# EarthyScience/EasyHybrid.jl

Hardware: NVIDIA B200
Metric: training samples/sec (fwd+bwd+Adam) (higher is better)
Workload: dtype f32

## Files before the change

easyhybrid.jl_b200/csrc/eh_epoch_kernel.cuh:

```cuda
#pragma once
#include "eh_step_kernel.cuh"

namespace eh {

struct EpochArgs {
    const float4* rec;
    const int* idx;
    long long n;
    int B;
    long long first_step;
    int nsteps;
    int nb;
    float* pblock;
    int nflat, ntheta;
    float* m;
    float* v;
    OptState* ost;
    const int* wsrc;
    const int* pmap;
    const int* cells;
    const float* pspan;
    const int* slot_of_flat;
    const float* bscal;
    uint2* pbuf;
    int pbuf_rows;
    unsigned tag_base;
    float* stats_out;
    int npartp;
    int work_floats;
    int wcomp;
    int pg_log2;
    int tile_floats;
    int T, agg_mean;
    int loss_kind[MAXT];
    PSlot slot[MAXPS];
    float pmc[4];
    int use_bn;
    const PmProgData* prog;
    int scale_rt;
    unsigned pass_mask[3];
    int pm_id;
    int opt_kind, adamw_coupled;
    float eta, beta1, beta2, eps, lambda;
    long long* dbg;
    const unsigned* ready;
    unsigned ready_base;
    unsigned* done;
    const int* host_total;
    float* loss_stream;
    long long batch_stride;
    int world, rank;
    unsigned step_base;
    uint2* inbox_peer[EH_MAX_WORLD];
    unsigned* err;
    int stagger_ns;
    int eng_off;
};

__device__ __forceinline__ void st_volatile_v2(uint2* p, unsigned x, unsigned y)
{
    asm volatile("st.volatile.global.v2.u32 [%0], {%1, %2};" ::"l"(p), "r"(x), "r"(y) : "memory");
}
__device__ __forceinline__ uint2 ld_volatile_v2(const uint2* p)
{
    uint2 v;
    asm volatile("ld.volatile.global.v2.u32 {%0, %1}, [%2];" : "=r"(v.x), "=r"(v.y) : "l"(p) : "memory");
    return v;
}
#ifndef EH_TOT_REPL_N
#define EH_TOT_REPL_N 8
#endif
constexpr int EH_TOT_REPL = EH_TOT_REPL_N;
constexpr int EH_PBUF_EXTRA_ROWS = 32;
constexpr unsigned EH_SPIN_LIMIT = 1u << 26;

__device__ __forceinline__ void st_cg_v4(uint2* p, unsigned x0, unsigned t0, unsigned x1, unsigned t1)
{
    asm volatile("st.global.cg.v4.u32 [%0], {%1, %2, %3, %4};" ::"l"(p), "r"(x0), "r"(t0), "r"(x1), "r"(t1) : "memory");
}
__device__ __forceinline__ uint4 ld_cg_v4(const uint2* p)
{
    uint4 v;
    asm volatile("ld.global.cg.v4.u32 {%0, %1, %2, %3}, [%4];" : "=r"(v.x), "=r"(v.y), "=r"(v.z), "=r"(v.w) : "l"(p) : "memory");
    return v;
}
__device__ __forceinline__ uint4 poll_pair_cg(const uint2* p, unsigned tag, unsigned* err)
{
    uint4 v = ld_cg_v4(p);
    unsigned spins = 0;
    while (v.y != tag || v.w != tag) {
        if (++spins > EH_SPIN_LIMIT) { *err = 1; break; }
        v = ld_cg_v4(p);
    }
    return v;
}
__device__ __forceinline__ void st_volatile_v4(uint2* p, unsigned x0, unsigned t0, unsigned x1, unsigned t1)
{
    asm volatile("st.volatile.global.v4.u32 [%0], {%1, %2, %3, %4};" ::"l"(p), "r"(x0), "r"(t0), "r"(x1), "r"(t1) : "memory");
}
__device__ __forceinline__ uint4 ld_volatile_v4(const uint2* p)
{
    uint4 v;
    asm volatile("ld.volatile.global.v4.u32 {%0, %1, %2, %3}, [%4];" : "=r"(v.x), "=r"(v.y), "=r"(v.z), "=r"(v.w) : "l"(p) : "memory");
    return v;
}

__device__ __forceinline__ uint4 poll_pair(const uint2* p, uint4 v, unsigned tag, unsigned* err)
{
    unsigned spins = 0;
    while (v.y != tag || v.w != tag) {
        if (++spins > EH_SPIN_LIMIT) { *err = 1; break; }
        v = ld_volatile_v4(p);
    }
    return v;
}

__device__ __forceinline__ float poll_slot(const uint2* p, unsigned tag, unsigned* err)
{
    uint2 v = ld_volatile_v2(p);
    unsigned spins = 0;
    while (v.y != tag) {
        if (++spins > EH_SPIN_LIMIT) { *err = 1; break; }
        v = ld_volatile_v2(p);
    }
    return __uint_as_float(v.x);
}

__device__ __forceinline__ void bar_sync_id(int id, int nthreads) { asm volatile("bar.sync %0, %1;" ::"r"(id), "r"(nthreads) : "memory"); }
__device__ __forceinline__ void bar_arrive_id(int id, int nthreads) { asm volatile("bar.arrive %0, %1;" ::"r"(id), "r"(nthreads) : "memory"); }

__device__ __forceinline__ void mbar_init(unsigned long long* bar, unsigned count)
{
    asm volatile("mbarrier.init.shared::cta.b64 [%0], %1;" ::"r"((unsigned)__cvta_generic_to_shared(bar)), "r"(count) : "memory");
}
__device__ __forceinline__ void mbar_expect_tx(unsigned long long* bar, unsigned bytes)
{
    asm volatile("mbarrier.arrive.expect_tx.shared::cta.b64 _, [%0], %1;" ::"r"((unsigned)__cvta_generic_to_shared(bar)), "r"(bytes) : "memory");
}
__device__ __forceinline__ void mbar_arrive(unsigned long long* bar)
{
    asm volatile("mbarrier.arrive.shared::cta.b64 _, [%0];" ::"r"((unsigned)__cvta_generic_to_shared(bar)) : "memory");
}
__device__ __forceinline__ bool mbar_try_wait(unsigned long long* bar, unsigned parity)
{
    unsigned ok;
    asm volatile(
        "{\n\t.reg .pred p;\n\t"
        "mbarrier.try_wait.parity.shared::cta.b64 p, [%1], %2;\n\t"
        "selp.u32 %0, 1, 0, p;\n\t}"
        : "=r"(ok) : "r"((unsigned)__cvta_generic_to_shared(bar)), "r"(parity) : "memory");
    return ok != 0;
}
__device__ __forceinline__ void mbar_wait(unsigned long long* bar, unsigned parity, unsigned* err, bool unbounded = false)
{
    unsigned spins = 0;
    while (!mbar_try_wait(bar, parity)) {
        if (!unbounded && ++spins > (1u << 22)) { *err = 1; break; }
    }
}
__device__ __forceinline__ void bulk_g2s(void* dst, const void* src, unsigned bytes, unsigned long long* bar)
{
    asm volatile("cp.async.bulk.shared::cluster.global.mbarrier::complete_tx::bytes [%0], [%1], %2, [%3];"
                 ::"r"((unsigned)__cvta_generic_to_shared(dst)), "l"(src), "r"(bytes), "r"((unsigned)__cvta_generic_to_shared(bar)) : "memory");
}

__device__ __forceinline__ void cta_chunk_range(int nchunks, int G, int bid, int& c0, int& cnt)
{
    const int base = nchunks / G, rem = nchunks - base * G;
    cnt = base + (bid < rem ? 1 : 0);
    c0 = bid * base + (bid < rem ? bid : rem);
}

__host__ __device__ constexpr int epoch_xbuf_floats(int npartp, int G) { return 4 * (npartp / 4 + G) + 8; }
__host__ __device__ constexpr int epoch_extra_floats(int npartp, int nflat, int tile_floats, int G)
{
    return npartp + 8 * rup4(nflat) + 2 * rup4(tile_floats) + 8 + epoch_xbuf_floats(npartp, G);
}

template <class E, class = void>
struct EngWpc { static constexpr int value = 1; };
template <class E>
struct EngWpc<E, decltype((void)E::WPC)> { static constexpr int value = E::WPC; };
template <class E>
constexpr int epoch_threads() { return EngWpc<E>::value > 1 ? (E::MAX_WARPS + 1) * 32 : ((E::MAX_WARPS + 1) * 32 > 512 ? 512 : (E::MAX_WARPS + 1) * 32); }

template <class E>
__global__ void __launch_bounds__(epoch_threads<E>(), 1) k_epoch(const EpochArgs a)
{
    constexpr int WPC = EngWpc<E>::value;
    using C = typename E::Cfg;
    extern __shared__ float4 smem4[];
    float* sW = reinterpret_cast<float*>(smem4);
    float* sS = sW + rup4(C::NW);
    const int lane = threadIdx.x & 31, warp = threadIdx.x >> 5, nwarps = blockDim.x >> 5;
    const int wcomp = a.wcomp;
    const bool service = warp == nwarps - 1;
    float* stage0 = sS + SS_FLOATS;
    float* stage = stage0 + (service ? 0 : warp) * E::STAGE_FLOATS;
    float* red = stage0 + a.work_floats;
    float* s_th = red + a.npartp;
    float* s_m = s_th + rup4(a.nflat);
    float* s_v = s_m + rup4(a.nflat);
    int* t_pmap = reinterpret_cast<int*>(s_v + rup4(a.nflat));
    int* t_cell0 = t_pmap + rup4(a.nflat);
    int* t_cell1 = t_cell0 + rup4(a.nflat);
    int* t_slot = t_cell1 + rup4(a.nflat);
    float* t_span = reinterpret_cast<float*>(t_slot + rup4(a.nflat));
    float4* tile0 = reinterpret_cast<float4*>(t_span + rup4(a.nflat));
    unsigned long long* mbar = reinterpret_cast<unsigned long long*>(reinterpret_cast<float*>(tile0) + 2 * rup4(a.tile_floats));
    unsigned* phi_flag = reinterpret_cast<unsigned*>(mbar + 2);
    float2* xbuf = reinterpret_cast<float2*>(phi_flag + 4);
    const int G = gridDim.x, bid = blockIdx.x;
    unsigned char* eng = reinterpret_cast<unsigned char*>(smem4) + a.eng_off;
    const int unit = warp / WPC, nunits = wcomp / WPC;
    if constexpr (WPC > 1) E::cta_init(eng);
    const bool tiles = a.tile_floats > 0;
    constexpr int R44 = C::R4 / 4;

    for (int p = threadIdx.x; p < a.nflat; p += blockDim.x) {
        s_th[p] = a.pblock[p];
        s_m[p] = a.m[p];
        s_v[p] = a.v[p];
        t_pmap[p] = a.pmap[p];
        t_cell0[p] = a.cells[2 * p];
        t_cell1[p] = a.cells[2 * p + 1];
        t_slot[p] = a.slot_of_flat[p];
        t_span[p] = a.pspan[p];
        if (p >= a.ntheta && p - a.ntheta < MAXPS) {
            const float sg0 = 1.f / (1.f + expf(-a.pblock[p]));
            sS[SS_SGD + p - a.ntheta] = a.pspan[p] * sg0 * (1.f - sg0);
        }
    }
    float b1t = a.ost->b1t, b2t = a.ost->b2t;
    long long tdone = 0, tskip = 0;
    if (threadIdx.x == 0) {
        mbar_init(&mbar[0], 1);
        mbar_init(&mbar[1], 1);
        *phi_flag = a.tag_base;
        phi_flag[1] = 0u;
        asm volatile("fence.mbarrier_init.release.cluster;" ::: "memory");
    }

    typename E::State st;
    if constexpr (WPC == 1) {
        if (!service) E::init_warp(st, stage, lane);
    }
    load_weights_and_scalars<C>(a.pblock, a.nflat, a.wsrc, nullptr, 0, sW, sS);
    __syncthreads();
    if constexpr (WPC > 1) {
        E::load_w2(eng, sW);
        asm volatile("fence.proxy.async.shared::cta;" ::: "memory");
        if (!service) E::init_warp(st, stage, lane, eng);
    }

    PmCtx cx;
    cx.pms = sS + SS_PMS;
    cx.c = a.pmc;
    cx.prog = a.prog;
    cx.scale_rt = a.scale_rt;
    for (int l = 0; l < 3; l++) cx.pass[l] = a.pass_mask[l];
    cx.uniform_mask = 0;
    cx.phi_flag = phi_flag;
    cx.phi_want = a.tag_base;
#pragma unroll
    for (int s = 0; s < MAXPS; s++)
        if (s >= C::NPS || a.slot[s].role != ROLE_NEURAL) cx.uniform_mask |= 1u << s;

    int bcur = (int)(a.first_step % a.nb);
    const int Blast = (int)(a.n - (long long)(a.nb - 1) * a.B);
    auto batch_size = [&](int b) { return b == a.nb - 1 ? Blast : a.B; };
    const long long bstride = a.batch_stride ? a.batch_stride : (long long)a.B;
    const bool stream = a.ready != nullptr;
    auto issue_tile = [&](int b, int buf) {
        const int Bk = batch_size(b);
        int c0, cnt;
        cta_chunk_range((Bk + E::CHUNK - 1) / E::CHUNK, G, bid, c0, cnt);
        const long long s0 = (long long)c0 * E::CHUNK;
        long long s1 = s0 + (long long)cnt * E::CHUNK;
        if (s1 > Bk) s1 = Bk;
        if (s1 > s0) {
            const unsigned bytes = (unsigned)(s1 - s0) * (unsigned)(C::R4 * 4);
            mbar_expect_tx(&mbar[buf], bytes);
            bulk_g2s(tile0 + (size_t)buf * (rup4(a.tile_floats) / 4), a.rec + ((long long)b * bstride + s0) * R44, bytes, &mbar[buf]);
        } else {
            mbar_arrive(&mbar[buf]);
        }
    };
    auto fetch_args = [&](int b, int buf) {
        FetchArgs fa;
        const int Bk = batch_size(b);
        fa.rec = a.rec;
        fa.idx = a.idx ? a.idx + (long long)b * a.B : nullptr;
        fa.rec_base = a.idx ? 0 : (long long)b * bstride;
        fa.B = Bk;
        fa.nchunks = (Bk + E::CHUNK - 1) / E::CHUNK;
        int c0, cnt;
        cta_chunk_range(fa.nchunks, G, bid, c0, cnt);
        fa.tile = tiles ? tile0 + (size_t)buf * (rup4(a.tile_floats) / 4) : nullptr;
        fa.tile_s0 = c0 * E::CHUNK;
        return fa;
    };
    auto load_bs = [&](int batch) {
        const float* bs = a.bscal + (size_t)batch * BS_STRIDE;
        float v = 0.f;
        if (lane < MAXT) v = bs[BS_C + lane];
        else if (lane < MAXT + 2 * C::P) v = a.use_bn ? bs[BS_BN + lane - MAXT] : (((lane - MAXT) & 1) ? 1.f : 0.f);
        else if (lane >= 28 && lane < 28 + MAXT) v = bs[BS_N + lane - 28];
        return v;
    };
    auto store_bs = [&](float v, int s) {
        if (lane < MAXT) sS[SS_C + lane] = v;
        else if (lane < MAXT + 2 * C::P) sS[SS_BN + lane - MAXT] = v;
        else if (lane >= 28 && lane < 28 + MAXT) sS[SS_NV2 + (s & 1) * MAXT + lane - 28] = v;
    };
    auto slot_ready = [&](int s, int batch) { return *reinterpret_cast<const volatile unsigned*>(a.ready + batch) == a.ready_base + (unsigned)s + 1u; };
    auto wait_slot = [&](int s, int batch) {
        for (;;) {
            if (slot_ready(s, batch)) return true;
            const int tot = *reinterpret_cast<const volatile int*>(a.host_total);
            if (tot > 0 && s >= tot) return false;
        }
    };
    volatile unsigned* stop_flag = phi_flag + 1;
    float pre = 0.f;
    bool have_next = false;
    if (service) {
        bool go = true;
        if (stream) go = wait_slot(0, bcur);
        if (go) {
            store_bs(load_bs(bcur), 0);
        } else if (lane == 0) {
            *stop_flag = 1u;
        }
    }
    __syncthreads();
    if (tiles && service && lane == 0 && !*stop_flag) issue_tile(bcur, 0);
    if (!tiles && !service) {
        const FetchArgs f0 = fetch_args(bcur, 0);
        int c0, cnt;
        cta_chunk_range(f0.nchunks, G, bid, c0, cnt);
        E::fetch(st, f0, unit < cnt ? c0 + unit : f0.nchunks, lane);
    }
#define EH_STAMP(slot)                                                                      \
    if (a.dbg && threadIdx.x == 0) a.dbg[((size_t)s * G + bid) * 32 + (slot)] = clock64();
#define EH_STAMP_SVC(slot)                                                                  \
    if (a.dbg && service && lane == 0) a.dbg[((size_t)s * G + bid) * 32 + (slot)] = clock64();

    const int NSL = a.npartp / 4;
    const int nown = (NSL - bid + G - 1) / G;
    const int ncomp_threads = wcomp * 32;
    const int Gp = (G + 3) & ~3;

    int s_end = a.nsteps;
    for (int s = 0; s < a.nsteps; s++) {
        if (*stop_flag) { s_end = s; break; }
        EH_STAMP(0)
        const int bnext = bcur + 1 == a.nb ? 0 : bcur + 1;
        const int par = s & 1;
        const unsigned tag = a.tag_base + (unsigned)s + 1u;
        uint2* part = a.pbuf + (size_t)par * a.pbuf_rows * a.npartp;
        uint2* tot = part + (size_t)(a.pbuf_rows - EH_TOT_REPL) * a.npartp;
        const uint2* mytot = tot + (size_t)(bid % EH_TOT_REPL) * a.npartp;

        if (service) {
            have_next = s + 1 < a.nsteps && (!stream || slot_ready(s + 1, bnext));
            if (have_next) {
                pre = load_bs(bnext);
                if (tiles && lane == 0) issue_tile(bnext, par ^ 1);
            }
        } else {
            const FetchArgs fa = fetch_args(bcur, par);
            const FetchArgs fn = fetch_args(bnext, par ^ 1);
            int c0, cnt, n0, ncnt;
            cta_chunk_range(fa.nchunks, G, bid, c0, cnt);
            cta_chunk_range(fn.nchunks, G, bid, n0, ncnt);
            const int nfirst = (s + 1 < a.nsteps && unit < ncnt) ? n0 + unit : fn.nchunks;
            E::step_begin(st, sW, lane);
            if (tiles) {
                mbar_wait(&mbar[par], (unsigned)(s >> 1) & 1u, a.err, stream);
                if (*stop_flag) { s_end = s; break; }
                E::fetch(st, fa, unit < cnt ? c0 + unit : fa.nchunks, lane);
            }
            cx.phi_want = a.tag_base + (unsigned)s;
            if constexpr (WPC > 1) {
                if (a.stagger_ns > 0 && unit > 0) __nanosleep((unsigned)(unit * a.stagger_ns));
            }
            for (int chunk = c0 + unit; chunk < c0 + cnt; chunk += nunits) {
                const bool last = chunk + nunits >= c0 + cnt;
                if constexpr (WPC > 1) {
                    if (last && !tiles) E::chunk(st, fn, nfirst, sW, sS, stage, lane, a.slot, a.loss_kind, cx, a.err);
                    else E::chunk(st, fa, last ? fa.nchunks : chunk + nunits, sW, sS, stage, lane, a.slot, a.loss_kind, cx, a.err);
                } else {
                    if (last && !tiles) E::chunk(st, fn, nfirst, sW, sS, stage, lane, a.slot, a.loss_kind, cx);
                    else E::chunk(st, fa, last ? fa.nchunks : chunk + nunits, sW, sS, stage, lane, a.slot, a.loss_kind, cx);
                }
            }
            if (a.dbg && lane == 0) a.dbg[((size_t)s * G + bid) * 32 + 8 + warp] = clock64();
            if (!tiles && unit >= cnt) E::fetch(st, fn, nfirst, lane);
            if constexpr (WPC > 1) E::reduce_prepare(st, stage0, a.err);
            else if (!E::SCRATCH_ALIASES_STAGE) E::reduce_prepare(st, stage0);
        }
        EH_STAMP(1)
        if constexpr (WPC == 1) {
            if (E::SCRATCH_ALIASES_STAGE) {
                __syncthreads();
                if (!service) E::reduce_prepare(st, stage0);
            }
        }
        __syncthreads();
        EH_STAMP(2)
        if (service && have_next) store_bs(pre, s + 1);

        for (int p0 = 0; p0 < a.npartp; p0 += blockDim.x) {
            const int p = p0 + threadIdx.x;
            const float v0 = p < E::NPART ? E::reduce_sum_at(stage0, wcomp, p) : 0.f;
            const float v1 = __shfl_down_sync(0xffffffffu, v0, 1);
            if (p < a.npartp && !(p & 1)) {
                const int k = p >> 1;
                if (G == 1) *reinterpret_cast<float2*>(red + p) = make_float2(v0, v1);
                else st_cg_v4(part + ((size_t)(k >> 1) * Gp + bid) * 4 + (k & 1) * 2, __float_as_uint(v0), tag, __float_as_uint(v1), tag);
            }
        }
        EH_STAMP(3)
        const float rb1 = 1.f / (1.f - b1t), rb2 = 1.f / (1.f - b2t);
        if (G > 1) {
            const int nitems = 2 * G * nown;
            for (int i = threadIdx.x; i < nitems; i += blockDim.x) {
                const int row = i / (2 * G), rem = i - row * 2 * G, half = rem & 1, peer = rem >> 1;
                const uint4 v = poll_pair_cg(part + (size_t)(bid + row * G) * Gp * 4 + rem * 2, tag, a.err);
                xbuf[(row * 2 + half) * G + peer] = make_float2(__uint_as_float(v.x), __uint_as_float(v.z));
            }
            __syncthreads();
            {
                const unsigned dtag = a.step_base + (unsigned)s + 1u;
                const int dpar = (int)((a.step_base + (unsigned)s) & 1u);
                for (int pr = nwarps - 1 - warp; pr < 2 * nown; pr += nwarps) {
                    EH_STAMP_SVC(24)
                    const float2* src = xbuf + (size_t)pr * G;
                    float acc0 = 0.f, acc1 = 0.f;
                    for (int c = lane; c < G; c += 32) { const float2 v = src[c]; acc0 += v.x; acc1 += v.y; }
                    for (int o = 16; o > 0; o >>= 1) {
                        acc0 += __shfl_xor_sync(0xffffffffu, acc0, o);
                        acc1 += __shfl_xor_sync(0xffffffffu, acc1, o);
                    }
                    const int ge = (bid + (pr >> 1) * G) * 4 + (pr & 1) * 2;
                    if (a.world > 1) {
                        float v0 = 0.f, v1 = 0.f;
                        if (lane < a.world) {
                            st_volatile_v4(a.inbox_peer[lane] + ((size_t)dpar * a.world + a.rank) * a.npartp + ge, __float_as_uint(acc0), dtag,
                                           __float_as_uint(acc1), dtag);
                            const uint2* in = a.inbox_peer[a.rank] + ((size_t)dpar * a.world + lane) * a.npartp + ge;
                            const uint4 v = poll_pair(in, ld_volatile_v4(in), dtag, a.err);
                            v0 = __uint_as_float(v.x);
                            v1 = __uint_as_float(v.z);
                        }
                        acc0 = 0.f; acc1 = 0.f;
                        for (int r = 0; r < a.world; r++) {
                            acc0 += __shfl_sync(0xffffffffu, v0, r);
                            acc1 += __shfl_sync(0xffffffffu, v1, r);
                        }
                    }
                    if (lane < EH_TOT_REPL) st_cg_v4(tot + (size_t)lane * a.npartp + ge, __float_as_uint(acc0), tag, __float_as_uint(acc1), tag);
                    EH_STAMP_SVC(25)
                }
            }
            for (int k = threadIdx.x; k < a.npartp / 2; k += blockDim.x) {
                const uint4 v = poll_pair_cg(mytot + 2 * k, tag, a.err);
                *reinterpret_cast<float2*>(red + 2 * k) = make_float2(__uint_as_float(v.x), __uint_as_float(v.z));
            }
        }
        __syncthreads();
        if (service) bar_arrive_id(1, blockDim.x);
        EH_STAMP(4)

        float ntot = 0.f, post = 1.f;
        for (int t = 0; t < a.T; t++) {
            const float nv = sS[SS_NV2 + par * MAXT + t];
            ntot += nv;
            if (a.loss_kind[t] == LOSS_RMSE) post = 1.f / (2.f * sqrtf(red[E::OFF_STATS + t] / nv));
        }
        const bool skip = ntot == 0.f;
        if (bid == 0 && service) {
            if (lane < MAXT) a.stats_out[(size_t)s * MAXT + lane] = red[E::OFF_STATS + lane];
            if (stream && lane == 0) {
                float L = 0.f;
                for (int t = 0; t < a.T; t++) {
                    const float nv = sS[SS_NV2 + par * MAXT + t], acc = red[E::OFF_STATS + t];
                    L += a.loss_kind[t] == LOSS_RMSE ? sqrtf(acc / nv) : acc / nv;
                }
                if (a.agg_mean) L /= (float)a.T;
                a.loss_stream[s] = skip ? __int_as_float(0x7fc00000) : L;
                *reinterpret_cast<volatile unsigned*>(a.done) = a.ready_base + (unsigned)s + 1u;
            }
        }
        const int pbeg = service ? a.ntheta + lane : threadIdx.x;
        const int pend = service ? a.nflat : a.ntheta;
        const int pstep = service ? 32 : ncomp_threads;
        if (!skip) {
            for (int p = pbeg; p < pend; p += pstep) {
                float g = red[t_pmap[p]] * post;
                float th = s_th[p];
                const bool phi_cached = p >= a.ntheta && p - a.ntheta < MAXPS;
                if (phi_cached) {
                    g *= sS[SS_SGD + p - a.ntheta];
                } else if (p >= a.ntheta) {
                    float sg = 1.f / (1.f + expf(-th));
                    g *= t_span[p] * sg * (1.f - sg);
                }
                float dx;
                if (a.opt_kind == OPT_ADAM || a.opt_kind == OPT_ADAMW) {
                    float mt = a.beta1 * s_m[p] + (1.f - a.beta1) * g;
                    float vt = a.beta2 * s_v[p] + (1.f - a.beta2) * g * g;
                    s_m[p] = mt;
                    s_v[p] = vt;
                    dx = mt * rb1 / (sqrtf(vt * rb2) + a.eps) * a.eta;
                    if (a.opt_kind == OPT_ADAMW) dx += (a.adamw_coupled ? a.eta * a.lambda : a.lambda) * th;
                } else if (a.opt_kind == OPT_RMSPROP) {
                    float qv = a.beta2 * s_v[p] + (1.f - a.beta2) * g * g;
                    s_v[p] = qv;
                    dx = g * a.eta / (sqrtf(qv) + a.eps);
                } else {
                    dx = a.eta * g;
                }
                th -= dx;
                s_th[p] = th;
                const int c0 = t_cell0[p], c1 = t_cell1[p];
                if (c0 >= 0) sW[c0] = th;
                if (c1 >= 0) sW[c1] = th;
                if constexpr (WPC > 1) {
                    if (c0 >= 0) E::patch_cell(eng, c0, th);
                    if (c1 >= 0) E::patch_cell(eng, c1, th);
                }
                if (p >= a.ntheta) {
                    const float sgn = 1.f / (1.f + expf(-th));
                    if (phi_cached) sS[SS_SGD + p - a.ntheta] = t_span[p] * sgn * (1.f - sgn);
                    const int sl = t_slot[p];
                    if (sl >= 0) {
                        const PSlot ps = a.slot[sl];
                        float val = ps.lo + ps.span * sgn;
                        float o4[4];
                        pm_prep_slot_fast(a.pm_id, sl, val, o4);
                        sS[SS_SLOT + sl] = val;
                        for (int i = 0; i < 4; i++) sS[SS_PMS + sl * PMS_PER_SLOT + i] = o4[i];
                    }
                }
            }
            b1t *= a.beta1;
            b2t *= a.beta2;
            tdone++;
        } else {
            tskip++;
        }
        EH_STAMP(5)
        if (service) {
            __syncwarp();
            __threadfence_block();
            if (lane == 0) asm volatile("st.volatile.shared.u32 [%0], %1;" ::"r"((unsigned)__cvta_generic_to_shared(phi_flag)), "r"(tag) : "memory");
            EH_STAMP_SVC(27)
            if (stream && !have_next && s + 1 < a.nsteps) {
                if (wait_slot(s + 1, bnext)) {
                    store_bs(load_bs(bnext), s + 1);
                    __syncwarp();
                    if (lane == 0) issue_tile(bnext, par ^ 1);
                } else {
                    if (lane == 0) {
                        *stop_flag = 1u;
                        __threadfence_block();
                        mbar_arrive(&mbar[par ^ 1]);
                    }
                    __syncwarp();
                }
            }
        }
        if (!service) {
            if constexpr (WPC > 1) asm volatile("fence.proxy.async.shared::cta;" ::: "memory");
            bar_sync_id(1, blockDim.x);
            E::after_reduce(st, stage, lane);
        }
        bcur = bnext;
        EH_STAMP(6)
    }
#undef EH_STAMP
#undef EH_STAMP_SVC

    __syncthreads();
    if constexpr (WPC > 1) E::cta_exit(eng);
    if (bid == 0) {
        for (int p = threadIdx.x; p < a.nflat; p += blockDim.x) {
            a.pblock[p] = s_th[p];
            a.m[p] = s_m[p];
            a.v[p] = s_v[p];
        }
        if (threadIdx.x < MAXPS) a.pblock[a.nflat + threadIdx.x] = sS[SS_SLOT + threadIdx.x];
        if (threadIdx.x < MAXPS * PMS_PER_SLOT) a.pblock[a.nflat + MAXPS + threadIdx.x] = sS[SS_PMS + threadIdx.x];
        if (threadIdx.x == 0) {
            a.ost->b1t = b1t;
            a.ost->b2t = b2t;
            a.ost->t += tdone;
            a.ost->skipped += tskip;
        }
    }
}

}
```

Baseline: 5.636 billion.

## Poll reduced gradient slots directly in optimizer loop instead of staging via shared

In the multi-block case, threads no longer copy the whole reduced-gradient totals buffer into shared memory and then wait on a block barrier. Each thread now polls only the global slots it needs, right at the point of use inside the optimizer loop and the loss/stats computation. Parameter state loads are hoisted so they can overlap with the poll. The aim is to remove one __syncthreads and a bulk copy from the critical path between the cross-block reduction and the Adam update, at the cost of more scattered per-element global polls. A step counter is also narrowed to int.

```diff
diff --git a/easyhybrid.jl_b200/csrc/eh_epoch_kernel.cuh b/easyhybrid.jl_b200/csrc/eh_epoch_kernel.cuh
--- a/easyhybrid.jl_b200/csrc/eh_epoch_kernel.cuh
+++ b/easyhybrid.jl_b200/csrc/eh_epoch_kernel.cuh
@@ -94,6 +94,21 @@
     }
     return v;
 }
+__device__ __forceinline__ uint2 ld_cg_v2(const uint2* p)
+{
+    uint2 v;
+    asm volatile("ld.global.cg.v2.u32 {%0, %1}, [%2];" : "=r"(v.x), "=r"(v.y) : "l"(p) : "memory");
+    return v;
+}
+__device__ __forceinline__ uint2 poll_slot_cg(const uint2* p, uint2 v, unsigned tag, unsigned* err)
+{
+    unsigned spins = 0;
+    while (v.y != tag) {
+        if (++spins > EH_SPIN_LIMIT) { *err = 1; break; }
+        v = ld_cg_v2(p);
+    }
+    return v;
+}
 __device__ __forceinline__ void st_volatile_v4(uint2* p, unsigned x0, unsigned t0, unsigned x1, unsigned t1)
 {
     asm volatile("st.volatile.global.v4.u32 [%0], {%1, %2, %3, %4};" ::"l"(p), "r"(x0), "r"(t0), "r"(x1), "r"(t1) : "memory");
@@ -232,7 +247,7 @@
         }
     }
     float b1t = a.ost->b1t, b2t = a.ost->b2t;
-    long long tdone = 0, tskip = 0;
+    int tdone = 0, tskip = 0;
     if (threadIdx.x == 0) {
         mbar_init(&mbar[0], 1);
         mbar_init(&mbar[1], 1);
@@ -464,33 +479,36 @@
                     EH_STAMP_SVC(25)
                 }
             }
-            for (int k = threadIdx.x; k < a.npartp / 2; k += blockDim.x) {
-                const uint4 v = poll_pair_cg(mytot + 2 * k, tag, a.err);
-                *reinterpret_cast<float2*>(red + 2 * k) = make_float2(__uint_as_float(v.x), __uint_as_float(v.z));
-            }
-        }
-        __syncthreads();
+        } else {
+            __syncthreads();
+        }
         if (service) bar_arrive_id(1, blockDim.x);
-        EH_STAMP(4)
-
+
+        auto total = [&](int e) {
+            if (G == 1) return red[e];
+            return __uint_as_float(poll_slot_cg(mytot + e, ld_cg_v2(mytot + e), tag, a.err).x);
+        };
         float ntot = 0.f, post = 1.f;
         for (int t = 0; t < a.T; t++) {
             const float nv = sS[SS_NV2 + par * MAXT + t];
             ntot += nv;
-            if (a.loss_kind[t] == LOSS_RMSE) post = 1.f / (2.f * sqrtf(red[E::OFF_STATS + t] / nv));
+            if (a.loss_kind[t] == LOSS_RMSE) post = 1.f / (2.f * sqrtf(total(E::OFF_STATS + t) / nv));
         }
         const bool skip = ntot == 0.f;
         if (bid == 0 && service) {
-            if (lane < MAXT) a.stats_out[(size_t)s * MAXT + lane] = red[E::OFF_STATS + lane];
-            if (stream && lane == 0) {
+            const float acc = lane < MAXT ? total(E::OFF_STATS + lane) : 0.f;
+            if (lane < MAXT) a.stats_out[(size_t)s * MAXT + lane] = acc;
+            if (stream) {
                 float L = 0.f;
                 for (int t = 0; t < a.T; t++) {
-                    const float nv = sS[SS_NV2 + par * MAXT + t], acc = red[E::OFF_STATS + t];
-                    L += a.loss_kind[t] == LOSS_RMSE ? sqrtf(acc / nv) : acc / nv;
+                    const float nv = sS[SS_NV2 + par * MAXT + t], acc_t = __shfl_sync(0xffffffffu, acc, t);
+                    L += a.loss_kind[t] == LOSS_RMSE ? sqrtf(acc_t / nv) : acc_t / nv;
                 }
                 if (a.agg_mean) L /= (float)a.T;
-                a.loss_stream[s] = skip ? __int_as_float(0x7fc00000) : L;
-                *reinterpret_cast<volatile unsigned*>(a.done) = a.ready_base + (unsigned)s + 1u;
+                if (lane == 0) {
+                    a.loss_stream[s] = skip ? __int_as_float(0x7fc00000) : L;
+                    *reinterpret_cast<volatile unsigned*>(a.done) = a.ready_base + (unsigned)s + 1u;
+                }
             }
         }
         const int pbeg = service ? a.ntheta + lane : threadIdx.x;
@@ -498,8 +516,13 @@
         const int pstep = service ? 32 : ncomp_threads;
         if (!skip) {
             for (int p = pbeg; p < pend; p += pstep) {
-                float g = red[t_pmap[p]] * post;
-                float th = s_th[p];
+                const int e = t_pmap[p];
+                uint2 gv = make_uint2(0u, 0u);
+                if (G > 1) gv = ld_cg_v2(mytot + e);
+                float th = s_th[p], m = s_m[p], v = s_v[p];
+                const int c0 = t_cell0[p], c1 = t_cell1[p];
+                float g = (G > 1 ? __uint_as_float(poll_slot_cg(mytot + e, gv, tag, a.err).x) : red[e]) * post;
+                EH_STAMP(4)
                 const bool phi_cached = p >= a.ntheta && p - a.ntheta < MAXPS;
                 if (phi_cached) {
                     g *= sS[SS_SGD + p - a.ntheta];
@@ -509,14 +532,14 @@
                 }
                 float dx;
                 if (a.opt_kind == OPT_ADAM || a.opt_kind == OPT_ADAMW) {
-                    float mt = a.beta1 * s_m[p] + (1.f - a.beta1) * g;
-                    float vt = a.beta2 * s_v[p] + (1.f - a.beta2) * g * g;
+                    float mt = a.beta1 * m + (1.f - a.beta1) * g;
+                    float vt = a.beta2 * v + (1.f - a.beta2) * g * g;
                     s_m[p] = mt;
                     s_v[p] = vt;
                     dx = mt * rb1 / (sqrtf(vt * rb2) + a.eps) * a.eta;
                     if (a.opt_kind == OPT_ADAMW) dx += (a.adamw_coupled ? a.eta * a.lambda : a.lambda) * th;
                 } else if (a.opt_kind == OPT_RMSPROP) {
-                    float qv = a.beta2 * s_v[p] + (1.f - a.beta2) * g * g;
+                    float qv = a.beta2 * v + (1.f - a.beta2) * g * g;
                     s_v[p] = qv;
                     dx = g * a.eta / (sqrtf(qv) + a.eps);
                 } else {
@@ -524,7 +547,6 @@
                 }
                 th -= dx;
                 s_th[p] = th;
-                const int c0 = t_cell0[p], c1 = t_cell1[p];
                 if (c0 >= 0) sW[c0] = th;
                 if (c1 >= 0) sW[c1] = th;
                 if constexpr (WPC > 1) {
```

Result: slower. 5.387 billion, median of 6 (-4.4%).
